# JuliaQuantumControl/Krotov.jl

Measured on NVIDIA B200. Metric: state_timesteps_per_s, higher is better.
Workload: dtype f64

## Files before the change

include/krotov_cuda.h:

```cpp
#ifndef KROTOV_CUDA_H
#define KROTOV_CUDA_H

#include <stdint.h>

#ifdef __cplusplus
extern "C" {
#endif

#define KROTOV_ABI_VERSION 1

typedef struct krotov_handle_s *krotov_handle;

enum krotov_status {
    KROTOV_OK = 0,
    KROTOV_ERR_ARG = 1,
    KROTOV_ERR_CUDA = 2,
    KROTOV_ERR_STATE = 3,
    KROTOV_ERR_UNSUPPORTED = 4,
    KROTOV_ERR_TIMEOUT = 5,
    KROTOV_ERR_NOMEM = 6
};

enum krotov_gen_format {
    KROTOV_GEN_DENSE_COLMAJOR = 0,
// ... 70 lines not shown
int krotov_create(const krotov_problem *problem, krotov_handle *out);
int krotov_destroy(krotov_handle h);
const char *krotov_last_error(krotov_handle h);
int krotov_get_info(krotov_handle h, krotov_info *out);

int krotov_set_cheby(krotov_handle h, int direction, int n_dt_class, const int32_t *dt_class_of_step,
                     const double *dt_of_class, const double *E_min, const double *Delta, const int32_t *m,
                     const double *coeffs, int m_max);

int krotov_set_amplitudes(krotov_handle h, int degree, const double *poly, const double *shape);

int krotov_forward(krotov_handle h, const double *pulses );

int krotov_set_chi(krotov_handle h, const double *chi );
int krotov_set_chi_coeffs(krotov_handle h, const double *coef);

int krotov_iterate(krotov_handle h, const double *guess_pulses, double *new_pulses, double *g_a_int);

int krotov_get_states(krotov_handle h, double *states );
int krotov_get_tau(krotov_handle h, double *tau );
int krotov_get_storage(krotov_handle h, int which, int k, int n0, int n1, double *out);

int krotov_get_profile(krotov_handle h, int cta, int64_t *out);

#define KROTOV_COMM_DESC_BYTES 256
int krotov_comm_export(krotov_handle h, void *desc );
int krotov_comm_connect(krotov_handle h, int rank, int world, const void *descs );

int krotov_group_connect(krotov_handle *handles, int world);
int krotov_group_iterate(krotov_handle *handles, int world, const double *guess_pulses, double *new_pulses,
                         double *g_a_int);

int krotov_hermitian_extremes(int n_mat, int d, const double *mats, double *e_min, double *e_max, int n_threads);
int krotov_envelope_extremes(int n_gen, int d, int n_ctrl, const double *H0, const double *Hc, int n_corner,
                             const double *amps, double *e_min, double *e_max, int n_threads);

int krotov_envelope_extremes_device(krotov_handle h, int n_corner, const double *amps, double *e_min, double *e_max);

#ifdef __cplusplus
}
#endif
#endif
```

krotov.jl_b200/_lib.py:

```python
from __future__ import annotations

import ctypes as C
import os

_HERE = os.path.dirname(os.path.abspath(__file__))
LIB_PATH = os.environ.get("KROTOV_CUDA_LIB") or os.path.join(_HERE, "libkrotov_cuda.so")

KROTOV_OK = 0
ERR_NAMES = {1: "KROTOV_ERR_ARG", 2: "KROTOV_ERR_CUDA", 3: "KROTOV_ERR_STATE", 4: "KROTOV_ERR_UNSUPPORTED",
             5: "KROTOV_ERR_TIMEOUT", 6: "KROTOV_ERR_NOMEM"}
GEN_DENSE_COLMAJOR, GEN_CSR = 0, 1
FORWARD, BACKWARD = 0, 1
CHI_HOST, CHI_SM, CHI_SS, CHI_RE = 0, 1, 2, 3
PATH_WARP, PATH_DENSE, PATH_SPARSE = 1, 2, 3
COMM_DESC_BYTES = 256

EXPORTS = [
    "krotov_abi_version", "krotov_create", "krotov_destroy", "krotov_last_error", "krotov_get_info",
    "krotov_set_cheby", "krotov_set_amplitudes", "krotov_forward", "krotov_set_chi", "krotov_set_chi_coeffs", "krotov_iterate",
    "krotov_get_states", "krotov_get_tau", "krotov_get_storage", "krotov_get_profile", "krotov_comm_export", "krotov_comm_connect",
    "krotov_group_connect", "krotov_group_iterate",
    "krotov_hermitian_extremes", "krotov_envelope_extremes", "krotov_envelope_extremes_device",
]


class KrotovCudaError(RuntimeError):
    def __init__(self, code, msg):
        super().__init__(f"libkrotov_cuda: {ERR_NAMES.get(code, code)}: {msg}")
        self.code = code
        self.detail = msg


class Problem(C.Structure):
    _fields_ = [
        ("struct_size", C.c_int32), ("d", C.c_int32), ("n_traj", C.c_int32), ("n_ctrl", C.c_int32),
        ("n_steps", C.c_int32), ("n_gen", C.c_int32), ("gen_format", C.c_int32), ("nnz", C.c_int32),
        ("tlist", C.c_void_p), ("gen_of_traj", C.c_void_p), ("csr_rowptr", C.c_void_p), ("csr_colind", C.c_void_p),
        ("gen_values", C.c_void_p), ("term_present", C.c_void_p), ("psi0", C.c_void_p), ("target", C.c_void_p),
        ("weight", C.c_void_p), ("update_shape", C.c_void_p), ("lambda_a", C.c_void_p),
        ("functional", C.c_int32), ("n_traj_global", C.c_int32), ("store_fw", C.c_int32), ("device", C.c_int32),
        ("force_path", C.c_int32), ("replicated_forward", C.c_int32), ("reserved", C.c_int32 * 6),
    ]

# ... 19 lines not shown
    if not os.path.exists(LIB_PATH):
        raise ImportError(
            f"{LIB_PATH} not found: the CUDA extension is not built. Run "
            "`python -c 'import __graft_entry__ as g; g.build()'` at the repo root. "
            "krotov_jl_b200 has no CPU fallback.")
    L = C.CDLL(LIB_PATH)
    vp, i32, dbl = C.c_void_p, C.c_int, C.c_double
    L.krotov_abi_version.restype = i32
    L.krotov_create.argtypes = [C.POINTER(Problem), C.POINTER(vp)]
    L.krotov_destroy.argtypes = [vp]
    L.krotov_last_error.argtypes = [vp]
    L.krotov_last_error.restype = C.c_char_p
    L.krotov_get_info.argtypes = [vp, C.POINTER(Info)]
    L.krotov_set_cheby.argtypes = [vp, i32, i32, vp, vp, vp, vp, vp, vp, i32]
    L.krotov_set_amplitudes.argtypes = [vp, i32, vp, vp]
    L.krotov_forward.argtypes = [vp, vp]
    L.krotov_set_chi.argtypes = [vp, vp]
    L.krotov_set_chi_coeffs.argtypes = [vp, vp]
    L.krotov_iterate.argtypes = [vp, vp, vp, vp]
    L.krotov_get_states.argtypes = [vp, vp]
    L.krotov_get_tau.argtypes = [vp, vp]
    L.krotov_get_storage.argtypes = [vp, i32, i32, i32, i32, vp]
    L.krotov_get_profile.argtypes = [vp, i32, vp]
    L.krotov_comm_export.argtypes = [vp, vp]
    L.krotov_comm_connect.argtypes = [vp, i32, i32, vp]
    L.krotov_group_connect.argtypes = [vp, i32]
    L.krotov_group_iterate.argtypes = [vp, i32, vp, vp, vp]
    L.krotov_hermitian_extremes.argtypes = [i32, i32, vp, vp, vp, i32]
    L.krotov_envelope_extremes.argtypes = [i32, i32, i32, vp, vp, i32, vp, vp, vp, i32]
    L.krotov_envelope_extremes_device.argtypes = [vp, i32, vp, vp, vp]
    for name in EXPORTS:
        if name not in ("krotov_last_error",):
            getattr(L, name).restype = i32
    L.krotov_last_error.restype = C.c_char_p
    _lib = L
    return L


def hermitian_extremes(stack, n_threads=0):
    import numpy as np

    a = np.ascontiguousarray(stack, np.complex128)
    n, d = a.shape[0], a.shape[-1]
    lo, hi = np.empty(n, np.float64), np.empty(n, np.float64)
    rc = lib().krotov_hermitian_extremes(n, d, a.ctypes.data_as(C.c_void_p), lo.ctypes.data_as(C.c_void_p),
                                         hi.ctypes.data_as(C.c_void_p), int(n_threads))
# ... 21 lines not shown
```

krotov.jl_b200/csrc/krotov_cuda.cu:

```cuda
#include <cuda_runtime.h>

#include <algorithm>
#include <chrono>
#include <cmath>
#include <complex>
#include <cstdio>
#include <cstdlib>
#include <cstring>
#include <map>
#include <set>
#include <string>
#include <vector>

#include <thread>

#include "../../include/krotov_cuda.h"
#include "dense_kernel.cuh"
#include "warp_kernel.cuh"
#include "warp2_kernel.cuh"
#include "tiny_kernel.cuh"
#include "kernel_table.h"

using cplx = std::complex<double>;

// ... 969 lines not shown
        if (h->has_target) {
            pad_states(pb->target, tmp);
            if ((rc = upload(h, h->d_target, tmp))) return bail(rc);
        }
        const size_t slab = (size_t)N * (N_T + 1) * h->lpt * 16;
        h->x_slab = slab / 16;
        if ((rc = dev_alloc(h, h->d_X, slab * (h->rf_wanted ? 2 : 1)))) return bail(rc);
        if (h->store_fw && (rc = dev_alloc(h, h->d_Phi, slab))) return bail(rc);
        if ((rc = dev_alloc(h, h->d_chiT, (size_t)N * h->lpt * 16))) return bail(rc);
        if ((rc = dev_alloc(h, h->d_psif, (size_t)N * h->lpt * 16))) return bail(rc);
        cudaMemcpy(h->d_psif.p, h->d_psi0.p, (size_t)N * h->lpt * 16, cudaMemcpyDeviceToDevice);
        if (h->has_target) {
            std::vector<cplx> tau0(N);
            const cplx *s0 = reinterpret_cast<const cplx *>(pb->psi0), *tg = reinterpret_cast<const cplx *>(pb->target);
            for (int k = 0; k < N; ++k) {
                cplx a(0, 0);
                for (int i = 0; i < d; ++i) a += std::conj(tg[(size_t)k * d + i]) * s0[(size_t)k * d + i];
                tau0[k] = a;
            }
            cudaMemcpy(h->d_tau.p, tau0.data(), (size_t)N * 16, cudaMemcpyHostToDevice);
        }
        h->swept = true;
        if ((rc = dev_alloc(h, h->d_R, ((size_t)N_T * h->nCTA * L + (size_t)N_T * L) * 8))) return bail(rc);
        if ((rc = dev_alloc(h, h->d_acc, (size_t)N_T * L * kr::kFixLimbs * 8))) return bail(rc);
        if (getenv("KROTOV_PROF")) {
            if ((rc = dev_alloc(h, h->d_prof, (size_t)h->nCTA * 8 * 8))) return bail(rc);
            cudaMemset(h->d_prof.p, 0, h->d_prof.bytes);
        }
    } else {
        kr::SparseDesc sd;
        if (path == KROTOV_PATH_SPARSE) {
            sd.W = hs.W; sd.nnz_union = hs.nnz_union; sd.hermitian = hs.hermitian;
            sd.cols = &hs.cols; sd.vals_f = &hs.vals_f; sd.vals_b = &hs.vals_b;
        }
        h->dense = kr::dense_create(h->d, h->N, h->L, h->N_T, h->n_gen, h->Hdense, h->gen_of_traj, pb->psi0,
                                    pb->target, h->store_fw, h->stream, h->err,
                                    path == KROTOV_PATH_SPARSE ? &sd : nullptr);
        if (!h->dense) return bail(KROTOV_ERR_UNSUPPORTED);
        std::vector<cplx>().swap(h->Hdense);
        if (!kr::dense_seed(h->dense, (double2 *)h->d_tau.p, h->err)) return bail(KROTOV_ERR_CUDA);
        h->swept = true;
    }
    if (cudaDeviceSynchronize() != cudaSuccess) return bail(fail(h, KROTOV_ERR_CUDA, "device sync after create failed"));
    *out = h;
    return KROTOV_OK;
}

int krotov_get_info(krotov_handle h, krotov_info *out) {
    if (!h || !out) return KROTOV_ERR_ARG;
// ... 537 lines not shown
            lo = std::min(lo, out[2 * ((size_t)g * n_corner + c)]);
            hi = std::max(hi, out[2 * ((size_t)g * n_corner + c) + 1]);
        }
        e_min[g] = lo;
        e_max[g] = hi;
    }
    return KROTOV_OK;
}

int krotov_get_profile(krotov_handle h, int cta, int64_t *out) {
    if (!h || !out) return KROTOV_ERR_ARG;
    for (int i = 0; i < 8; ++i) out[i] = 0;
    if (!h->d_prof.p) return fail(h, KROTOV_ERR_STATE, "profiling counters are off (set KROTOV_PROF=1 before krotov_create)");
    cudaSetDevice(h->device);
    std::vector<long long> tmp((size_t)h->nCTA * 8);
    KR_CUDA(h, cudaMemcpy(tmp.data(), h->d_prof.p, tmp.size() * 8, cudaMemcpyDeviceToHost));
    if (cta >= h->nCTA) return fail(h, KROTOV_ERR_ARG, "cta out of range");
    for (int c = 0; c < h->nCTA; ++c)
        if (cta < 0 || c == cta)
            for (int i = 0; i < 8; ++i) out[i] = std::max<int64_t>(out[i], tmp[(size_t)c * 8 + i]);
    return KROTOV_OK;
}

struct CommDesc {
    cudaIpcMemHandle_t mh[2];
    cudaIpcMemHandle_t xh;
};
struct CommDescTail {
    int nCTA;
    int n_traj, n_traj_global;
    int rf_ok;
};
static_assert(sizeof(CommDesc) + sizeof(CommDescTail) <= KROTOV_COMM_DESC_BYTES, "descriptor too large");

int krotov_comm_export(krotov_handle h, void *desc) {
    if (!h || !desc) return KROTOV_ERR_ARG;
    cudaSetDevice(h->device);
    CommDesc cd;
    memset(&cd, 0, sizeof(cd));
    for (int par = 0; par < 2; ++par) KR_CUDA(h, cudaIpcGetMemHandle(&cd.mh[par], h->d_mbox[par].p));
    if (h->path == KROTOV_PATH_WARP) KR_CUDA(h, cudaIpcGetMemHandle(&cd.xh, h->d_X.p));
    memset(desc, 0, KROTOV_COMM_DESC_BYTES);
    memcpy(desc, &cd, sizeof(cd));
    CommDescTail tail{h->path == KROTOV_PATH_WARP ? h->nCTA : 0, h->N, h->N_global, rf_eligible(h) ? 1 : 0};
    memcpy((char *)desc + sizeof(cd), &tail, sizeof(tail));
    return KROTOV_OK;
// ... 61 lines not shown
```

krotov.jl_b200/csrc/warp2_kernel.cuh:

```cuda
#pragma once
#include "warp_kernel.cuh"

namespace kr {

template <int W>
__device__ __forceinline__ void row_dot2(const double2 (&g)[W + 1], const int (&col)[W], const double2 *__restrict__ va,
                                         const double2 *__restrict__ vb, const double2 owna, const double2 ownb,
                                         double &ara, double &aia, double &arb, double &aib) {
    double ra1 = 0.0, ia1 = 0.0, rb1 = 0.0, ib1 = 0.0;
    ara = fma(g[W].x, owna.x, ara);
    ra1 = fma(-g[W].y, owna.y, ra1);
    aia = fma(g[W].x, owna.y, aia);
    ia1 = fma(g[W].y, owna.x, ia1);
    arb = fma(g[W].x, ownb.x, arb);
    rb1 = fma(-g[W].y, ownb.y, rb1);
    aib = fma(g[W].x, ownb.y, aib);
    ib1 = fma(g[W].y, ownb.x, ib1);
#pragma unroll
    for (int s = 0; s < W; ++s) {
        const double2 xa = va[col[s]];
        const double2 xb = vb[col[s]];
        ara = fma(g[s].x, xa.x, ara);
        ra1 = fma(-g[s].y, xa.y, ra1);
        aia = fma(g[s].x, xa.y, aia);
// ... 157 lines not shown
    StepMeta fmeta = load_meta(p.dtc_f, p.m_f, p.phase_f, p.coef_f, p.ndtc_f, p.mmax_f, gi, 0);
    double2 chia = make_double2(0.0, 0.0), chib = make_double2(0.0, 0.0);
    if (p.mode == 1 && live) {
        chia = p.X[(size_t)ka * (N_T + 1) * 32 + lane];
        chib = p.X[(size_t)kb * (N_T + 1) * 32 + lane];
    }
    long long t_wait_b = 0, t_overlap = 0, t_step = 0;
    for (int n = 0; n < N_T; ++n) {
        double eps[LT];
        const long long ts0 = clock64();
        if (p.mode == 1) {
            double part[LT];
#pragma unroll
            for (int l = 0; l < LT; ++l) part[l] = 0.0;
            if (live) {
#pragma unroll
                for (int l = 0; l < LT; ++l) {
                    double war = 0.0, wai = 0.0, wbr = 0.0, wbi = 0.0;
                    row_dot2<W>(P[l + 1], col, myps, myps + 32, pa, pb, war, wai, wbr, wbi);
                    part[l] = fma(inv_s, fma(chia.x, war, chia.y * wai), part[l]);
                    part[l] = fma(inv_s, fma(chib.x, wbr, chib.y * wbi), part[l]);
                }
            }
#pragma unroll
            for (int l = 0; l < LT; ++l) red[(size_t)l * wpc * 32 + warp * 32 + lane] = part[l];
            bar_arrive(1, nthr_all);
            const long long w0 = clock64();
            t_overlap += w0 - ts0;
            if (n + 1 < N_T && live) {
                chia = p.X[((size_t)ka * (N_T + 1) + n + 1) * 32 + lane];
                chib = p.X[((size_t)kb * (N_T + 1) + n + 1) * 32 + lane];
            }
            bar_sync(2, nthr_all);
#pragma unroll
            for (int l = 0; l < LT; ++l) eps[l] = eps_s[l];
            if (p.prof != nullptr) {
                asm volatile("" ::"d"(eps[0]) : "memory");
                t_wait_b += clock64() - w0;
            }
        } else {
#pragma unroll
            for (int l = 0; l < LT; ++l) eps[l] = p.amp_old[(size_t)l * N_T + n];
        }
        const StepMeta fmeta_next =
            load_meta(p.dtc_f, p.m_f, p.phase_f, p.coef_f, p.ndtc_f, p.mmax_f, gi, n + 1 < N_T ? n + 1 : n);
        if (live) {
#pragma unroll
            for (int s = 0; s <= W; ++s) g[s] = P[0][s];
// ... 56 lines not shown
```

krotov.jl_b200/csrc/warp_kernel.cuh:

```cuda
#pragma once
#include <cuda_runtime.h>
#include <stdint.h>

namespace kr {

constexpr int kMaxRanks = 8;
constexpr int kMaxCtrl = 8;
constexpr int kAmpMaxDeg = 4;
constexpr unsigned long long kSentinel = 0xFFFFFFFFFFFFFFFFull;

struct WarpParams {
    int d, N, L, N_T, n_gen;
    int wpc;
    int tpw;
    int nCTA;
    int mode;
    int mu_hermitian;
    int store_fw;
    int ndtc_f, ndtc_b, mmax_f, mmax_b;
    const int *gen_of_traj;
    const int *cols;
    const double2 *Pf, *Pb;
    const double *inv_s_f;
    const double *coef_f, *coef_b;
// ... 279 lines not shown

__device__ __forceinline__ void poll_broadcast(const double *E, const int L, const int lane, double (&tot)[kMaxCtrl],
                                               int *err_flag, const long long timeout) {
    const long long t0 = clock64();
    int spins = 0;
    unsigned long long u;
    for (;;) {
        u = ld_poll_u64<false>(E + (lane < L ? lane : 0));
        if (__all_sync(0xffffffffu, u != kSentinel)) break;
        if ((++spins & 63) == 0) {
            if (clock64() - t0 > timeout || *(volatile int *)err_flag) {
                atomicExch(err_flag, 1);
                break;
            }
        }
    }
    const double v = __longlong_as_double((long long)u);
#pragma unroll
    for (int l = 0; l < kMaxCtrl; ++l) tot[l] = __shfl_sync(0xffffffffu, v, l < L ? l : 0);
}


constexpr int kFixFrac = 88, kFixLimbBits = 40, kFixLimbs = 3, kFixBiasBit = 119;

__device__ __forceinline__ bool fix_from_double(const double x, unsigned __int128 &biased, const int lim_exp = 31) {
    const unsigned long long bits = (unsigned long long)__double_as_longlong(fabs(x));
    const int ebits = (int)(bits >> 52);
    if (ebits >= 1023 + lim_exp) return false;
    const unsigned long long mant = (bits & 0xFFFFFFFFFFFFFull) | (ebits ? (1ull << 52) : 0ull);
    const int shift = (ebits ? ebits : 1) - 1075 + kFixFrac;
    unsigned __int128 mag = 0;
    if (shift >= 0)
        mag = (unsigned __int128)mant << shift;
    else if (shift > -64)
        mag = mant >> (-shift);
    const unsigned __int128 bias = (unsigned __int128)1 << kFixBiasBit;
    biased = (x < 0.0) ? bias - mag : bias + mag;
    return true;
}

__device__ __forceinline__ double fix_to_double(const unsigned long long w0, const unsigned long long w1,
                                                const unsigned long long w2, const int n) {
    const unsigned long long mask = (1ull << 48) - 1;
    unsigned __int128 sum = (unsigned __int128)(w0 & mask) + ((unsigned __int128)(w1 & mask) << kFixLimbBits) +
                            ((unsigned __int128)(w2 & mask) << (2 * kFixLimbBits));
    const unsigned __int128 bias = (unsigned __int128)n << kFixBiasBit;
    const bool neg = sum < bias;
    const unsigned __int128 mag = neg ? bias - sum : sum - bias;
    const unsigned long long hi = (unsigned long long)(mag >> 64), lo = (unsigned long long)mag;
    double d;
    if (hi == 0) {
        d = __ull2double_rn(lo);
    } else {
        const int sh = 64 - __clzll((long long)hi);
        unsigned long long top = (sh == 64) ? hi : ((hi << (64 - sh)) | (lo >> sh));
        const unsigned long long lost = (sh == 64) ? lo : (lo << (64 - sh));
        if (lost) top |= 1ull;
        d = scalbn(__ull2double_rn(top), sh);
    }
    d = scalbn(d, -kFixFrac);
    return neg ? -d : d;
}

__device__ __forceinline__ void red_add_u64(unsigned long long *p, unsigned long long v) {
    asm volatile("red.relaxed.gpu.global.add.u64 [%0], %1;" ::"l"(p), "l"(v) : "memory");
}

__device__ __forceinline__ bool atomic_grid_sum(unsigned long long *An, const int nCTA, const int L, const int lane,
                                                double (&tot)[kMaxCtrl], int *err_flag, const long long timeout,
                                                const bool wait = true) {
    const int nw = L * kFixLimbs;
    const int myl = lane / kFixLimbs, myj = lane - myl * kFixLimbs;
    double mine = 0.0;
#pragma unroll
    for (int l = 0; l < kMaxCtrl; ++l)
        if (l == myl) mine = tot[l];
    if (lane < nw) {
        unsigned __int128 v;
        const bool ok = fix_from_double(mine, v);
        unsigned long long add = 1ull << 56;
        if (ok)
            add += (unsigned long long)(v >> (myj * kFixLimbBits)) & ((1ull << kFixLimbBits) - 1);
        else
            add += 1ull << 48;
        red_add_u64(An + lane, add);
    }
    if (!wait) return true;
    const long long t0 = clock64();
    int spins = 0;
    unsigned long long w = 0;
    for (;;) {
        if (lane < nw) w = ld_poll_u64<false>(reinterpret_cast<const double *>(An + lane));
        const bool pending = lane < nw && (int)(w >> 56) != nCTA;
        if (!__any_sync(0xffffffffu, pending)) break;
        if ((++spins & 63) == 0) {
            if (clock64() - t0 > timeout || *(volatile int *)err_flag) {
                atomicExch(err_flag, 1);
                break;
            }
        }
    }
    const bool misfit = lane < nw && ((w >> 48) & 0xFF) != 0;
    if (__any_sync(0xffffffffu, misfit)) return false;
    const int src = (lane < L ? lane : 0) * kFixLimbs;
    const unsigned long long w0 = __shfl_sync(0xffffffffu, w, src), w1 = __shfl_sync(0xffffffffu, w, src + 1),
                             w2 = __shfl_sync(0xffffffffu, w, src + 2);
    const double du = fix_to_double(w0, w1, w2, nCTA);
#pragma unroll
    for (int l = 0; l < kMaxCtrl; ++l) tot[l] = __shfl_sync(0xffffffffu, du, l < L ? l : 0);
    return true;
}

constexpr int kXLimbBits = 30, kXLimbs = 4, kXBiasBit = 116, kXMisShift = 41, kXCntShift = 52, kXMaxArrivals = 2047;

__device__ __forceinline__ bool fixx_from_double(const double x, unsigned __int128 &biased) {
    const unsigned long long bits = (unsigned long long)__double_as_longlong(fabs(x));
    const int ebits = (int)(bits >> 52);
    if (ebits >= 1023 + (kXBiasBit - kFixFrac)) return false;
    const unsigned long long mant = (bits & 0xFFFFFFFFFFFFFull) | (ebits ? (1ull << 52) : 0ull);
    const int shift = (ebits ? ebits : 1) - 1075 + kFixFrac;
    unsigned __int128 mag = 0;
    if (shift >= 0)
        mag = (unsigned __int128)mant << shift;
    else if (shift > -64)
        mag = mant >> (-shift);
    const unsigned __int128 bias = (unsigned __int128)1 << kXBiasBit;
    biased = (x < 0.0) ? bias - mag : bias + mag;
    return true;
}

__device__ __forceinline__ double fix_mag_to_double(const unsigned __int128 mag, const bool neg) {
    const unsigned long long hi = (unsigned long long)(mag >> 64), lo = (unsigned long long)mag;
    double d;
    if (hi == 0) {
        d = __ull2double_rn(lo);
    } else {
        const int sh = 64 - __clzll((long long)hi);
        unsigned long long top = (sh == 64) ? hi : ((hi << (64 - sh)) | (lo >> sh));
        const unsigned long long lost = (sh == 64) ? lo : (lo << (64 - sh));
        if (lost) top |= 1ull;
        d = scalbn(__ull2double_rn(top), sh);
    }
    d = scalbn(d, -kFixFrac);
    return neg ? -d : d;
}

__device__ __forceinline__ void red_add_sys_u64(unsigned long long *p, unsigned long long v) {
    asm volatile("red.relaxed.sys.global.add.u64 [%0], %1;" ::"l"(p), "l"(v) : "memory");
}

__device__ __forceinline__ bool xrank_atomic_sum(const WarpParams &p, const int n, const int L, const int lane,
                                                 double (&tot)[kMaxCtrl]) {
    const int nw = L * kXLimbs;
    const int myl = lane / kXLimbs, myj = lane - myl * kXLimbs;
    double mine = 0.0;
#pragma unroll
    for (int l = 0; l < kMaxCtrl; ++l)
        if (l == myl) mine = tot[l];
    const size_t off = ((size_t)n * nw + (lane < nw ? lane : 0)) * (size_t)p.xacc_stride;
    if (lane < nw) {
        unsigned __int128 v;
        const bool ok = fixx_from_double(mine, v);
        unsigned long long add = 1ull << kXCntShift;
        if (ok)
            add += (unsigned long long)(v >> (myj * kXLimbBits)) & ((1ull << kXLimbBits) - 1);
        else
            add += 1ull << kXMisShift;
// ... 16 lines not shown
                atomicExch(p.err_flag, 1);
                break;
            }
        }
    }
    const bool misfit = lane < nw && ((w >> kXMisShift) & 0x7FF) != 0;
    if (__any_sync(0xffffffffu, misfit)) return false;
    const int src = (lane < L ? lane : 0) * kXLimbs;
    const unsigned long long mask = (1ull << kXMisShift) - 1;
    unsigned __int128 sum = 0;
#pragma unroll
    for (int j = 0; j < kXLimbs; ++j)
        sum += (unsigned __int128)(__shfl_sync(0xffffffffu, w, src + j) & mask) << (j * kXLimbBits);
    const unsigned __int128 bias = (unsigned __int128)p.total_ctas << kXBiasBit;
    const bool neg = sum < bias;
    const double du = fix_mag_to_double(neg ? bias - sum : sum - bias, neg);
#pragma unroll
    for (int l = 0; l < kMaxCtrl; ++l) tot[l] = __shfl_sync(0xffffffffu, du, l < L ? l : 0);
    return true;
}

constexpr int kHSumBits = 52, kHMisShift = 52, kHCntShift = 56, kHLimExp = 28;

__device__ __forceinline__ unsigned long long atom_add_u64(unsigned long long *p, unsigned long long v) {
    unsigned long long old;
    asm volatile("atom.relaxed.gpu.global.add.u64 %0, [%1], %2;" : "=l"(old) : "l"(p), "l"(v) : "memory");
    return old;
}

__device__ __forceinline__ bool xrank_hier_sum(const WarpParams &p, const int n, const int L, const int lane,
                                               double (&tot)[kMaxCtrl]) {
    const int nw = L * kFixLimbs;
    const int myl = lane / kFixLimbs, myj = lane - myl * kFixLimbs;
    double mine = 0.0;
#pragma unroll
    for (int l = 0; l < kMaxCtrl; ++l)
        if (l == myl) mine = tot[l];
    const bool by_store = p.xchg_hier == 2;
    const size_t widx = ((size_t)n * L + (lane < nw ? myl : 0)) * kXLimbs + (lane < nw ? myj : 0);
    const size_t off = by_store ? widx * kMaxRanks : widx * (size_t)p.xacc_stride;
    if (lane < nw) {
        unsigned __int128 v;
        const bool ok = fix_from_double(mine, v, kHLimExp);
        unsigned long long add = 1ull << 56;
        if (ok)
            add += (unsigned long long)(v >> (myj * kFixLimbBits)) & ((1ull << kFixLimbBits) - 1);
        else
            add += 1ull << 48;
        unsigned long long total = add;
        if (p.nCTA > 1) total += atom_add_u64(p.acc + (size_t)n * nw + lane, add);
        if ((int)(total >> 56) == p.nCTA) {
            unsigned long long fwd = 1ull << kHCntShift;
            if ((total >> 48) & 0xFF)
                fwd += 1ull << kHMisShift;
            else
                fwd += total & ((1ull << 48) - 1);
            for (int i = 1; i <= p.world; ++i) {
                int r = p.rank + i;
                if (r >= p.world) r -= p.world;
                if (by_store)
                    asm volatile("st.relaxed.sys.global.u64 [%0], %1;" ::"l"(p.xacc[r] + off + p.rank), "l"(fwd) : "memory");
                else
                    red_add_sys_u64(p.xacc[r] + off, fwd);
            }
        }
    }
    const long long t0 = clock64();
    int spins = 0;
    unsigned long long w = 0;
    const double *mine_p = reinterpret_cast<const double *>(p.xacc[p.rank] + off);
    for (;;) {
        bool pending = false;
        if (lane < nw) {
// ... 42 lines not shown
    double tot[kMaxCtrl];
#pragma unroll
    for (int l = 0; l < kMaxCtrl; ++l) tot[l] = tot_io[l];
    bool summed = false, acc_used = false;
    if (p.xacc[0] != nullptr) {
        if (p.xchg_hier) {
            summed = xrank_hier_sum(p, n, L, lane, tot);
            acc_used = true;
        } else {
            summed = xrank_atomic_sum(p, n, L, lane, tot);
        }
        if (!summed && cta == 0 && lane == 0) atomicAdd(p.err_flag + 1, 1);
    }
    if (!summed) {
        double *Rn = p.R + (size_t)n * L * p.nCTA;
        const bool use_acc = p.acc != nullptr && p.nCTA > 1 && !acc_used;
        if (p.nCTA > 1) {
#pragma unroll
            for (int l = 0; l < kMaxCtrl; ++l)
                if (l < L && lane == l) st_relaxed_gpu_f64(Rn + (size_t)l * p.nCTA + cta, tot[l]);
        }
        bool have_rank_sum = p.nCTA == 1;
        if (use_acc)
            have_rank_sum = atomic_grid_sum(p.acc + (size_t)n * L * kFixLimbs, p.nCTA, L, lane, tot, p.err_flag,
                                            p.timeout_cycles, cta == 0);
        const size_t off = (size_t)n * L * p.world;
        if (cta == 0) {
            if (!have_rank_sum) {
                if (use_acc && lane == 0) atomicAdd(p.err_flag + 1, 1);
                reducer_gather<false>(Rn, p.nCTA, L, lane, gbuf, tot, p.err_flag, p.timeout_cycles);
            }
#pragma unroll
            for (int l = 0; l < kMaxCtrl; ++l)
                if (l < L && lane < p.world) st_relaxed_f64(p.mbox[lane] + off + (size_t)l * p.world + p.rank, tot[l]);
        }
        if (p.mbox_all || p.nCTA == 1) {
            reducer_gather<true>(p.mbox[p.rank] + off, p.world, L, lane, gbuf, tot, p.err_flag, p.timeout_cycles);
        } else {
            double *En = p.E + (size_t)n * L;
            if (cta == 0) {
                reducer_gather<true>(p.mbox[p.rank] + off, p.world, L, lane, gbuf, tot, p.err_flag, p.timeout_cycles);
#pragma unroll
                for (int l = 0; l < kMaxCtrl; ++l)
                    if (l < L && lane == l) st_relaxed_gpu_f64(En + l, tot[l]);
            } else {
                poll_broadcast(En, L, lane, tot, p.err_flag, p.timeout_cycles);
            }
// ... 19 lines not shown
    } else {
#pragma unroll
        for (int l = 0; l < kMaxCtrl; ++l)
            if (l < L && lane == l) st_relaxed_gpu_f64(Rn + (size_t)l * p.nCTA, tot[l]);
        reducer_gather<false>(Rn, p.nCTA, L, lane, gbuf, tot, p.err_flag, p.timeout_cycles);
#pragma unroll
        for (int l = 0; l < kMaxCtrl; ++l)
            if (l < L && lane == l) st_relaxed_gpu_f64(En + l, tot[l]);
    }
#pragma unroll
    for (int l = 0; l < kMaxCtrl; ++l) tot_io[l] = tot[l];
}

static __device__ __noinline__ double amp_eval_cold(const WarpParams *pp, const int l, const double e, const double shp) {
    double c = e;
    if (pp->amp_poly != nullptr) {
        const double *q = pp->amp_poly + l * (kAmpMaxDeg + 1);
        c = q[kAmpMaxDeg];
#pragma unroll
        for (int d = kAmpMaxDeg - 1; d >= 0; --d) c = fma(c, e, q[d]);
    }
    if (pp->amp_shape != nullptr) c = __dmul_rn(shp, c);
    return c;
}

__device__ __forceinline__ void comm_warp_run(const WarpParams &p, const int cta, const int L, const int lane, const int wpc,
                                              const int nthr_all, double *red, double *eps_s, double *gbuf,
                                              WarpParams *p_sh) {
    const int N_T = p.N_T;
    if (p.mode != 1) return;
    {
        const unsigned long long *src = reinterpret_cast<const unsigned long long *>(&p);
        unsigned long long *dst = reinterpret_cast<unsigned long long *>(p_sh);
        for (int i = lane; i < (int)(sizeof(WarpParams) / 8); i += 32) dst[i] = src[i];
        __syncwarp();
    }
    double ga = 0.0;
    const bool nonlin = p.amp_dfac != nullptr;
    long long c_wait_a = 0, c_reduce = 0, c_gather = 0;
    for (int n = 0; n < N_T; ++n) {
        double a_ln = 0.0, e_old = 0.0, dtn = 0.0, dfac = 1.0, shp = 1.0, a_eff = 0.0;
        if (lane < L) {
            a_ln = p.alpha[(size_t)lane * N_T + n];
            e_old = p.eps_old[(size_t)lane * N_T + n];
            dtn = p.dt[n];
            a_eff = a_ln;
            if (nonlin) {
                dfac = p.amp_dfac[(size_t)lane * N_T + n];
                if (p.amp_shape != nullptr) shp = p.amp_shape[(size_t)lane * N_T + n];
                a_eff = __dmul_rn(a_ln, dfac);
            }
        }
        const long long c0 = clock64();
        bar_sync(1, nthr_all);
        const long long c1 = clock64();
        double tot[kMaxCtrl];
#pragma unroll
        for (int l = 0; l < kMaxCtrl; ++l) {
            double sacc = 0.0;
            if (l < L)
                for (int q = 0; q < wpc; ++q) sacc += red[(size_t)l * wpc * 32 + q * 32 + lane];
            tot[l] = sacc;
        }
#pragma unroll
        for (int o = 16; o > 0; o >>= 1) {
#pragma unroll
            for (int l = 0; l < kMaxCtrl; ++l)
                if (l < L) tot[l] += __shfl_xor_sync(0xffffffffu, tot[l], o);
        }
        const long long c2 = clock64();
        bool summed = p.nCTA == 1 && p.world == 1;
        if (p.world > 1) {
            double tl[kMaxCtrl];
#pragma unroll
            for (int l = 0; l < kMaxCtrl; ++l) tl[l] = tot[l];
            exchange_ranks(p_sh, cta, n, L, lane, tl, gbuf);
#pragma unroll
            for (int l = 0; l < kMaxCtrl; ++l) tot[l] = tl[l];
            summed = true;
        } else if (p.acc != nullptr && p.nCTA > 1) {
            summed = atomic_grid_sum(p.acc + (size_t)n * L * kFixLimbs, p.nCTA, L, lane, tot, p.err_flag, p.timeout_cycles);
            if (!summed && cta == 0 && lane == 0) atomicAdd(p.err_flag + 1, 1);
        }
        if (!summed) {
            double tl[kMaxCtrl];
#pragma unroll
            for (int l = 0; l < kMaxCtrl; ++l) tl[l] = tot[l];
            exchange_gather(p_sh, cta, n, L, lane, tl, gbuf);
#pragma unroll
            for (int l = 0; l < kMaxCtrl; ++l) tot[l] = tl[l];
        }
        const long long c3 = clock64();
        c_wait_a += c1 - c0;
        c_reduce += c2 - c1;
        c_gather += c3 - c2;
        double mine = 0.0;
#pragma unroll
        for (int l = 0; l < kMaxCtrl; ++l)
            if (lane == l) mine = tot[l];
        double e_new = 0.0;
        if (lane < L) {
            const double d_eps = __dmul_rn(a_eff, mine);
            e_new = __dadd_rn(e_old, d_eps);
            double c_new = e_new;
            if (nonlin) c_new = amp_eval_cold(p_sh, lane, e_new, shp);
            eps_s[lane] = c_new;
        }
        bar_arrive(2, nthr_all);
        if (cta == 0 && lane < L) {
            p.eps_new[(size_t)lane * N_T + n] = e_new;
            const double du = nonlin ? __dmul_rn(dfac, mine) : mine;
            ga = __dadd_rn(ga, __dmul_rn(__dmul_rn(a_ln, __dmul_rn(fabs(du), fabs(du))), dtn));
        }
    }
    if (cta == 0 && lane < L) p.g_a_int[lane] = ga;
    if (p.prof != nullptr && lane == 0) {
        p.prof[cta * 8 + 3] = c_wait_a;
        p.prof[cta * 8 + 4] = c_reduce;
        p.prof[cta * 8 + 5] = c_gather;
    }
}

static __device__ __noinline__ void rf_forward_records(const WarpParams *pp, const double2 *rf_ring, unsigned long long *rf_bar,
                                                       int *rf_prog, const int cta, const int warp, const int lane,
                                                       const int n_prod, const int n_fwd) {
    const WarpParams &p = *pp;
    const int N_T = p.N_T, wpc = p.wpc, world = p.rf_world, nCTA = p.nCTA, bw_lo = p.bw_lo;
    const long long timeout = p.timeout_cycles;
    double2 *Xr[kMaxRanks];
#pragma unroll
    for (int r = 0; r < kMaxRanks; ++r) Xr[r] = p.Xr[r];
// ... 318 lines not shown
                const int k = kbase + t;
                if (k >= p.N) break;
                const int gi = (t == 0) ? g0 : p.gen_of_traj[k];
                const double inv_s = (t == 0) ? inv_s0 : p.inv_s_f[gi];
                const double2 psi = (tpw == 1) ? psi_reg : mypsi[t * LPT + lane];
                const double2 chi = (t == 0) ? chi_next : p.X[((size_t)k * (N_T + 1) + n) * LPT + lane];
                if (PREG) {
#pragma unroll
                    for (int l = 0; l < NT - 1; ++l) {
                        double wr = 0.0, wi = 0.0;
                        row_dot<W>(P[l + 1], col, mypsi + t * LPT, psi, wr, wi);
                        part[l] = fma(inv_s, fma(chi.x, wr, chi.y * wi), part[l]);
                    }
                } else {
                    const double2 *Pg = p.Pf + (size_t)gi * (1 + L) * rowstride;
                    for (int l = 0; l < L; ++l) {
                        load_row<W, LPT>(Pg + (size_t)(l + 1) * rowstride, g, lane);
                        double wr = 0.0, wi = 0.0;
                        row_dot<W>(g, col, mypsi + t * LPT, psi, wr, wi);
                        part[l] = fma(inv_s, fma(chi.x, wr, chi.y * wi), part[l]);
                    }
                }
            }
#pragma unroll
            for (int l = 0; l < (PREG ? LT : kMaxCtrl); ++l)
                if (l < L) red[(size_t)l * wpc * LPT + warp * LPT + lane] = part[l];
            bar_arrive(1, nthr_all);
            const long long w0 = clock64();
            t_overlap += w0 - ts0;
            if (n + 1 < N_T && k0 < p.N) chi_next = p.X[((size_t)k0 * (N_T + 1) + n + 1) * LPT + lane];
            if (PREG && FAST && k0 < p.N) {
#pragma unroll
                for (int q = 0; q < NT; ++q) {
                    double wr = 0.0, wi = 0.0;
                    row_dot<W>(P[q], col, mypsi, psi_reg, wr, wi);
                    wv[q] = make_double2(wr, wi);
                }
                chibuf[lane] = chi_next;
                grp_sync<LPT>(gbar);
#pragma unroll
                for (int l = 0; l < NT - 1; ++l) {
                    double wr = 0.0, wi = 0.0;
                    row_dot<W>(P[l + 1], col, chibuf, chi_next, wr, wi);
                    xi[l] = make_double2(wr, wi);
                }
                grp_sync<LPT>(gbar);
            }
            bar_sync(2, nthr_all);
#pragma unroll
            for (int l = 0; l < (PREG ? LT : kMaxCtrl); ++l)
                if (l < L) eps[l] = eps_s[l];
            if (p.prof != nullptr) {
                asm volatile("" ::"d"(eps[0]) : "memory");
                t_wait_b += clock64() - w0;
            }
        } else {
#pragma unroll
            for (int l = 0; l < (PREG ? LT : kMaxCtrl); ++l)
                if (l < L) eps[l] = p.amp_old[(size_t)l * N_T + n];
        }
        const StepMeta fmeta_next =
            load_meta(p.dtc_f, p.m_f, p.phase_f, p.coef_f, p.ndtc_f, p.mmax_f, g0, n + 1 < N_T ? n + 1 : n);
        for (int t = 0; t < tpw; ++t) {
            const int k = kbase + t;
            if (k >= p.N) break;
            const int gi = (t == 0) ? g0 : p.gen_of_traj[k];
            const StepMeta sm = (t == 0) ? fmeta : load_meta(p.dtc_f, p.m_f, p.phase_f, p.coef_f, p.ndtc_f, p.mmax_f, gi, n);
            if (PREG) {
#pragma unroll
                for (int s = 0; s <= W; ++s) g[s] = P[0][s];
#pragma unroll
                for (int l = 0; l < NT - 1; ++l) {
#pragma unroll
                    for (int s = 0; s <= W; ++s) {
                        g[s].x = fma(eps[l], P[l + 1][s].x, g[s].x);
                        g[s].y = fma(eps[l], P[l + 1][s].y, g[s].y);
                    }
// ... 80 lines not shown
```

krotov.jl_b200/engine.py:

```python
from __future__ import annotations

import ctypes as C

import numpy as np

from . import _lib as B


def _ptr(a):
    return None if a is None else a.ctypes.data_as(C.c_void_p)


class KrotovCuda:
    def __init__(self, *, tlist, H0, Hc, gen_of_traj, psi0, target=None, weight=None, update_shape, lambda_a,
                 functional=B.CHI_HOST, n_traj_global=0, store_fw=False, device=0, force_path=0, csr=False,
                 replicated_forward=False):
        lib = B.lib()
        self._lib = lib
        self._h = C.c_void_p()
        tlist = np.ascontiguousarray(tlist, np.float64)
        psi0 = np.ascontiguousarray(psi0, np.complex128)
        N, d = psi0.shape
        n_gen = len(H0)
        L = len(Hc[0])
# ... 133 lines not shown
    def tau(self):
        out = np.empty(self.N, np.complex128)
        self._check(self._lib.krotov_get_tau(self._h, _ptr(out)))
        return out

    def storage(self, which, k, n0=0, n1=None):
        n1 = self.N_T + 1 if n1 is None else n1
        out = np.empty((n1 - n0, self.d), np.complex128)
        self._check(self._lib.krotov_get_storage(self._h, int(which), int(k), int(n0), int(n1), _ptr(out)))
        return out

    def envelope_extremes(self, corners):
        amps = np.ascontiguousarray(corners, np.float64).reshape(-1, self.L)
        lo, hi = np.empty(self.n_gen, np.float64), np.empty(self.n_gen, np.float64)
        self._check(self._lib.krotov_envelope_extremes_device(self._h, amps.shape[0], _ptr(amps), _ptr(lo), _ptr(hi)))
        return lo, hi

    def profile(self, cta=-1):
        out = np.zeros(8, np.int64)
        self._check(self._lib.krotov_get_profile(self._h, int(cta), _ptr(out)))
        names = ["backward", "forward", "wait_pulse", "comm_wait_partials", "comm_reduce", "comm_gather", "overlap", "fw_step_total"]
        return dict(zip(names, out.tolist()))

    def comm_export(self):
        buf = (C.c_ubyte * B.COMM_DESC_BYTES)()
        self._check(self._lib.krotov_comm_export(self._h, buf))
        return bytes(buf)

    def comm_connect(self, rank, world, descs):
        blob = b"".join(descs)
        assert len(blob) == world * B.COMM_DESC_BYTES
        buf = (C.c_ubyte * len(blob)).from_buffer_copy(blob)
        self._check(self._lib.krotov_comm_connect(self._h, int(rank), int(world), buf))


class KrotovCudaGroup:

    def __init__(self, engines, bounds, gens, replicated=False):
        self.engines, self.bounds, self.gens = list(engines), list(bounds), [np.asarray(g, int) for g in gens]
        self.replicated = bool(replicated)
        e0 = self.engines[0]
        self._lib = e0._lib
        self.N = e0.N if replicated else sum(e.N for e in self.engines)
        self.d, self.L, self.N_T = e0.d, e0.L, e0.N_T
        self.n_gen = len(self.gens[0]) if replicated else sum(len(g) for g in self.gens)
        self.world = len(self.engines)
# ... 85 lines not shown
```

Measured before the change: 333.5 million.

## Warp-reduce partials before handoff and poll limbs directly in grid sum

Worker warps now reduce their per-control partials with warp shuffles before writing them to shared memory. The comm warp therefore sums one value per warp instead of 32 lanes per warp, and its trailing shuffle reduction is removed. The atomic grid sum has each lane poll its own three limbs directly rather than having many lanes poll and then shuffle, and the final broadcast is skipped where it is not needed. A per-step timeline profiler gated by KROTOV_PROF is also added; it adds clock reads when enabled and makes some parts of the code path differ from the unprofiled one.

```diff
diff --git a/include/krotov_cuda.h b/include/krotov_cuda.h
--- a/include/krotov_cuda.h
+++ b/include/krotov_cuda.h
@@ -116,6 +116,7 @@
 int krotov_get_storage(krotov_handle h, int which, int k, int n0, int n1, double *out);
 
 int krotov_get_profile(krotov_handle h, int cta, int64_t *out);
+int krotov_get_step_timeline(krotov_handle h, int64_t *out);
 
 #define KROTOV_COMM_DESC_BYTES 256
 int krotov_comm_export(krotov_handle h, void *desc );
diff --git a/krotov.jl_b200/_lib.py b/krotov.jl_b200/_lib.py
--- a/krotov.jl_b200/_lib.py
+++ b/krotov.jl_b200/_lib.py
@@ -18,7 +18,7 @@
 EXPORTS = [
     "krotov_abi_version", "krotov_create", "krotov_destroy", "krotov_last_error", "krotov_get_info",
     "krotov_set_cheby", "krotov_set_amplitudes", "krotov_forward", "krotov_set_chi", "krotov_set_chi_coeffs", "krotov_iterate",
-    "krotov_get_states", "krotov_get_tau", "krotov_get_storage", "krotov_get_profile", "krotov_comm_export", "krotov_comm_connect",
+    "krotov_get_states", "krotov_get_tau", "krotov_get_storage", "krotov_get_profile", "krotov_get_step_timeline", "krotov_comm_export", "krotov_comm_connect",
     "krotov_group_connect", "krotov_group_iterate",
     "krotov_hermitian_extremes", "krotov_envelope_extremes", "krotov_envelope_extremes_device",
 ]
@@ -84,6 +84,7 @@
     L.krotov_get_tau.argtypes = [vp, vp]
     L.krotov_get_storage.argtypes = [vp, i32, i32, i32, i32, vp]
     L.krotov_get_profile.argtypes = [vp, i32, vp]
+    L.krotov_get_step_timeline.argtypes = [vp, vp]
     L.krotov_comm_export.argtypes = [vp, vp]
     L.krotov_comm_connect.argtypes = [vp, i32, i32, vp]
     L.krotov_group_connect.argtypes = [vp, i32]
diff --git a/krotov.jl_b200/csrc/krotov_cuda.cu b/krotov.jl_b200/csrc/krotov_cuda.cu
--- a/krotov.jl_b200/csrc/krotov_cuda.cu
+++ b/krotov.jl_b200/csrc/krotov_cuda.cu
@@ -1015,9 +1015,9 @@
         }
         h->swept = true;
         if ((rc = dev_alloc(h, h->d_R, ((size_t)N_T * h->nCTA * L + (size_t)N_T * L) * 8))) return bail(rc);
-        if ((rc = dev_alloc(h, h->d_acc, (size_t)N_T * L * kr::kFixLimbs * 8))) return bail(rc);
+        if ((rc = dev_alloc(h, h->d_acc, (size_t)N_T * kr::acc_step_words(L) * 8))) return bail(rc);
         if (getenv("KROTOV_PROF")) {
-            if ((rc = dev_alloc(h, h->d_prof, (size_t)h->nCTA * 8 * 8))) return bail(rc);
+            if ((rc = dev_alloc(h, h->d_prof, (size_t)h->nCTA * (8 + kr::kTlSamples * kr::kTlSlots) * 8))) return bail(rc);
             cudaMemset(h->d_prof.p, 0, h->d_prof.bytes);
         }
     } else {
@@ -1601,6 +1601,15 @@
     return KROTOV_OK;
 }
 
+int krotov_get_step_timeline(krotov_handle h, int64_t *out) {
+    if (!h || !out) return KROTOV_ERR_ARG;
+    if (!h->d_prof.p) return fail(h, KROTOV_ERR_STATE, "profiling counters are off (set KROTOV_PROF=1 before krotov_create)");
+    cudaSetDevice(h->device);
+    const size_t n = (size_t)h->nCTA * kr::kTlSamples * kr::kTlSlots;
+    KR_CUDA(h, cudaMemcpy(out, (const long long *)h->d_prof.p + (size_t)h->nCTA * 8, n * 8, cudaMemcpyDeviceToHost));
+    return KROTOV_OK;
+}
+
 struct CommDesc {
     cudaIpcMemHandle_t mh[2];
     cudaIpcMemHandle_t xh;
diff --git a/krotov.jl_b200/csrc/warp2_kernel.cuh b/krotov.jl_b200/csrc/warp2_kernel.cuh
--- a/krotov.jl_b200/csrc/warp2_kernel.cuh
+++ b/krotov.jl_b200/csrc/warp2_kernel.cuh
@@ -203,8 +203,7 @@
                     part[l] = fma(inv_s, fma(chib.x, wbr, chib.y * wbi), part[l]);
                 }
             }
-#pragma unroll
-            for (int l = 0; l < LT; ++l) red[(size_t)l * wpc * 32 + warp * 32 + lane] = part[l];
+            hand_over_partials(part, LT, red, wpc, warp, lane);
             bar_arrive(1, nthr_all);
             const long long w0 = clock64();
             t_overlap += w0 - ts0;
diff --git a/krotov.jl_b200/csrc/warp_kernel.cuh b/krotov.jl_b200/csrc/warp_kernel.cuh
--- a/krotov.jl_b200/csrc/warp_kernel.cuh
+++ b/krotov.jl_b200/csrc/warp_kernel.cuh
@@ -325,6 +325,14 @@
 
 
 constexpr int kFixFrac = 88, kFixLimbBits = 40, kFixLimbs = 3, kFixBiasBit = 119;
+constexpr int kAccWordStride = 1;
+__host__ __device__ constexpr size_t acc_step_words(const int L) { return (size_t)L * kFixLimbs * kAccWordStride; }
+
+constexpr int kTlEvery = 16, kTlSamples = 128, kTlSlots = 16;
+__device__ __forceinline__ long long *tl_record(const WarpParams &p, const int cta, const int n) {
+    if (p.prof == nullptr || n % kTlEvery != 0 || n / kTlEvery >= kTlSamples) return nullptr;
+    return p.prof + (size_t)p.nCTA * 8 + ((size_t)cta * kTlSamples + n / kTlEvery) * kTlSlots;
+}
 
 __device__ __forceinline__ bool fix_from_double(const double x, unsigned __int128 &biased, const int lim_exp = 31) {
     const unsigned long long bits = (unsigned long long)__double_as_longlong(fabs(x));
@@ -342,6 +350,20 @@
     return true;
 }
 
+__device__ __forceinline__ double fix_mag_to_double(const unsigned __int128 mag, const bool neg) {
+    const unsigned long long hi = (unsigned long long)(mag >> 64), lo = (unsigned long long)mag;
+    const int sh = hi ? 64 - __clzll((long long)hi) : 0;
+    unsigned long long top = lo;
+    if (sh == 64) {
+        top = hi | (lo != 0 ? 1ull : 0ull);
+    } else if (sh > 0) {
+        top = (hi << (64 - sh)) | (lo >> sh);
+        if (lo << (64 - sh)) top |= 1ull;
+    }
+    const double d = __ull2double_rn(top) * __longlong_as_double((long long)(1023 + sh - kFixFrac) << 52);
+    return neg ? -d : d;
+}
+
 __device__ __forceinline__ double fix_to_double(const unsigned long long w0, const unsigned long long w1,
                                                 const unsigned long long w2, const int n) {
     const unsigned long long mask = (1ull << 48) - 1;
@@ -349,35 +371,29 @@
                             ((unsigned __int128)(w2 & mask) << (2 * kFixLimbBits));
     const unsigned __int128 bias = (unsigned __int128)n << kFixBiasBit;
     const bool neg = sum < bias;
-    const unsigned __int128 mag = neg ? bias - sum : sum - bias;
-    const unsigned long long hi = (unsigned long long)(mag >> 64), lo = (unsigned long long)mag;
-    double d;
-    if (hi == 0) {
-        d = __ull2double_rn(lo);
-    } else {
-        const int sh = 64 - __clzll((long long)hi);
-        unsigned long long top = (sh == 64) ? hi : ((hi << (64 - sh)) | (lo >> sh));
-        const unsigned long long lost = (sh == 64) ? lo : (lo << (64 - sh));
-        if (lost) top |= 1ull;
-        d = scalbn(__ull2double_rn(top), sh);
-    }
-    d = scalbn(d, -kFixFrac);
-    return neg ? -d : d;
+    return fix_mag_to_double(neg ? bias - sum : sum - bias, neg);
 }
 
 __device__ __forceinline__ void red_add_u64(unsigned long long *p, unsigned long long v) {
     asm volatile("red.relaxed.gpu.global.add.u64 [%0], %1;" ::"l"(p), "l"(v) : "memory");
 }
 
+__device__ __forceinline__ unsigned long long atom_add_u64(unsigned long long *p, unsigned long long v) {
+    unsigned long long old;
+    asm volatile("atom.relaxed.gpu.global.add.u64 %0, [%1], %2;" : "=l"(old) : "l"(p), "l"(v) : "memory");
+    return old;
+}
+
 __device__ __forceinline__ bool atomic_grid_sum(unsigned long long *An, const int nCTA, const int L, const int lane,
                                                 double (&tot)[kMaxCtrl], int *err_flag, const long long timeout,
-                                                const bool wait = true) {
+                                                const bool wait = true, const bool bcast = true, long long *tl = nullptr) {
     const int nw = L * kFixLimbs;
     const int myl = lane / kFixLimbs, myj = lane - myl * kFixLimbs;
     double mine = 0.0;
 #pragma unroll
     for (int l = 0; l < kMaxCtrl; ++l)
         if (l == myl) mine = tot[l];
+    unsigned long long prev = 0;
     if (lane < nw) {
         unsigned __int128 v;
         const bool ok = fix_from_double(mine, v);
@@ -386,15 +402,24 @@
             add += (unsigned long long)(v >> (myj * kFixLimbBits)) & ((1ull << kFixLimbBits) - 1);
         else
             add += 1ull << 48;
-        red_add_u64(An + lane, add);
-    }
+        if (tl != nullptr && lane == 0)
+            prev = atom_add_u64(An, add);
+        else
+            red_add_u64(An + lane * kAccWordStride, add);
+    }
+    if (tl != nullptr && lane == 0) tl[2] = clock64();
     if (!wait) return true;
+    const int src = lane < L ? lane * kFixLimbs : 0;
     const long long t0 = clock64();
     int spins = 0;
-    unsigned long long w = 0;
+    unsigned long long w0 = 0, w1 = 0, w2 = 0;
     for (;;) {
-        if (lane < nw) w = ld_poll_u64<false>(reinterpret_cast<const double *>(An + lane));
-        const bool pending = lane < nw && (int)(w >> 56) != nCTA;
+        if (lane < L) {
+            w0 = ld_poll_u64<false>(reinterpret_cast<const double *>(An + (src + 0) * kAccWordStride));
+            w1 = ld_poll_u64<false>(reinterpret_cast<const double *>(An + (src + 1) * kAccWordStride));
+            w2 = ld_poll_u64<false>(reinterpret_cast<const double *>(An + (src + 2) * kAccWordStride));
+        }
+        const bool pending = lane < L && ((int)(w0 >> 56) != nCTA || (int)(w1 >> 56) != nCTA || (int)(w2 >> 56) != nCTA);
         if (!__any_sync(0xffffffffu, pending)) break;
         if ((++spins & 63) == 0) {
             if (clock64() - t0 > timeout || *(volatile int *)err_flag) {
@@ -403,14 +428,15 @@
             }
         }
     }
-    const bool misfit = lane < nw && ((w >> 48) & 0xFF) != 0;
+    if (tl != nullptr && lane == 0) {
+        tl[3] = clock64();
+        tl[5] = (long long)(prev >> 56);
+    }
+    const bool misfit = lane < L && (((w0 | w1 | w2) >> 48) & 0xFF) != 0;
     if (__any_sync(0xffffffffu, misfit)) return false;
-    const int src = (lane < L ? lane : 0) * kFixLimbs;
-    const unsigned long long w0 = __shfl_sync(0xffffffffu, w, src), w1 = __shfl_sync(0xffffffffu, w, src + 1),
-                             w2 = __shfl_sync(0xffffffffu, w, src + 2);
     const double du = fix_to_double(w0, w1, w2, nCTA);
 #pragma unroll
-    for (int l = 0; l < kMaxCtrl; ++l) tot[l] = __shfl_sync(0xffffffffu, du, l < L ? l : 0);
+    for (int l = 0; l < kMaxCtrl; ++l) tot[l] = bcast ? __shfl_sync(0xffffffffu, du, l < L ? l : 0) : du;
     return true;
 }
 
@@ -430,22 +456,6 @@
     const unsigned __int128 bias = (unsigned __int128)1 << kXBiasBit;
     biased = (x < 0.0) ? bias - mag : bias + mag;
     return true;
-}
-
-__device__ __forceinline__ double fix_mag_to_double(const unsigned __int128 mag, const bool neg) {
-    const unsigned long long hi = (unsigned long long)(mag >> 64), lo = (unsigned long long)mag;
-    double d;
-    if (hi == 0) {
-        d = __ull2double_rn(lo);
-    } else {
-        const int sh = 64 - __clzll((long long)hi);
-        unsigned long long top = (sh == 64) ? hi : ((hi << (64 - sh)) | (lo >> sh));
-        const unsigned long long lost = (sh == 64) ? lo : (lo << (64 - sh));
-        if (lost) top |= 1ull;
-        d = scalbn(__ull2double_rn(top), sh);
-    }
-    d = scalbn(d, -kFixFrac);
-    return neg ? -d : d;
 }
 
 __device__ __forceinline__ void red_add_sys_u64(unsigned long long *p, unsigned long long v) {
@@ -508,12 +518,6 @@
 
 constexpr int kHSumBits = 52, kHMisShift = 52, kHCntShift = 56, kHLimExp = 28;
 
-__device__ __forceinline__ unsigned long long atom_add_u64(unsigned long long *p, unsigned long long v) {
-    unsigned long long old;
-    asm volatile("atom.relaxed.gpu.global.add.u64 %0, [%1], %2;" : "=l"(old) : "l"(p), "l"(v) : "memory");
-    return old;
-}
-
 __device__ __forceinline__ bool xrank_hier_sum(const WarpParams &p, const int n, const int L, const int lane,
                                                double (&tot)[kMaxCtrl]) {
     const int nw = L * kFixLimbs;
@@ -534,7 +538,7 @@
         else
             add += 1ull << 48;
         unsigned long long total = add;
-        if (p.nCTA > 1) total += atom_add_u64(p.acc + (size_t)n * nw + lane, add);
+        if (p.nCTA > 1) total += atom_add_u64(p.acc + (size_t)n * acc_step_words(L) + lane * kAccWordStride, add);
         if ((int)(total >> 56) == p.nCTA) {
             unsigned long long fwd = 1ull << kHCntShift;
             if ((total >> 48) & 0xFF)
@@ -623,7 +627,7 @@
         }
         bool have_rank_sum = p.nCTA == 1;
         if (use_acc)
-            have_rank_sum = atomic_grid_sum(p.acc + (size_t)n * L * kFixLimbs, p.nCTA, L, lane, tot, p.err_flag,
+            have_rank_sum = atomic_grid_sum(p.acc + (size_t)n * acc_step_words(L), p.nCTA, L, lane, tot, p.err_flag,
                                             p.timeout_cycles, cta == 0);
         const size_t off = (size_t)n * L * p.world;
         if (cta == 0) {
@@ -689,6 +693,31 @@
     }
     if (pp->amp_shape != nullptr) c = __dmul_rn(shp, c);
     return c;
+}
+
+template <int NL>
+__device__ __forceinline__ void hand_over_partials(double (&part)[NL], const int L, double *red, const int nw32,
+                                                   const int hw, const int lane32) {
+    if constexpr (NL == kMaxCtrl) {
+        for (int l = 0; l < L; ++l) {
+            double v = part[l];
+#pragma unroll
+            for (int o = 16; o > 0; o >>= 1) v += __shfl_xor_sync(0xffffffffu, v, o);
+            if (lane32 == 0) red[(size_t)l * nw32 + hw] = v;
+        }
+    } else {
+#pragma unroll
+        for (int o = 16; o > 0; o >>= 1) {
+#pragma unroll
+            for (int l = 0; l < NL; ++l)
+                if (l < L) part[l] += __shfl_xor_sync(0xffffffffu, part[l], o);
+        }
+        if (lane32 == 0) {
+#pragma unroll
+            for (int l = 0; l < NL; ++l)
+                if (l < L) red[(size_t)l * nw32 + hw] = part[l];
+        }
+    }
 }
 
 __device__ __forceinline__ void comm_warp_run(const WarpParams &p, const int cta, const int L, const int lane, const int wpc,
@@ -718,24 +747,36 @@
                 a_eff = __dmul_rn(a_ln, dfac);
             }
         }
+        long long *const rec = tl_record(p, cta, n);
         const long long c0 = clock64();
         bar_sync(1, nthr_all);
         const long long c1 = clock64();
+        if (rec != nullptr) {
+            const double x = red[0];
+            asm volatile("" ::"d"(x) : "memory");
+            if (lane == 0) rec[0] = clock64();
+        }
         double tot[kMaxCtrl];
 #pragma unroll
         for (int l = 0; l < kMaxCtrl; ++l) {
             double sacc = 0.0;
-            if (l < L)
-                for (int q = 0; q < wpc; ++q) sacc += red[(size_t)l * wpc * 32 + q * 32 + lane];
+            if (l < L) {
+                const double *r = red + (size_t)l * wpc;
+                for (int q0 = 0; q0 < wpc; q0 += 8) {
+                    double v[8];
+#pragma unroll
+                    for (int j = 0; j < 8; ++j) v[j] = (q0 + j < wpc) ? r[q0 + j] : 0.0;
+#pragma unroll
+                    for (int j = 0; j < 8; ++j) sacc += v[j];
+                }
+            }
             tot[l] = sacc;
         }
-#pragma unroll
-        for (int o = 16; o > 0; o >>= 1) {
-#pragma unroll
-            for (int l = 0; l < kMaxCtrl; ++l)
-                if (l < L) tot[l] += __shfl_xor_sync(0xffffffffu, tot[l], o);
-        }
         const long long c2 = clock64();
+        if (rec != nullptr && lane == 0) {
+            asm volatile("" ::"d"(tot[0]) : "memory");
+            rec[1] = clock64();
+        }
         bool summed = p.nCTA == 1 && p.world == 1;
         if (p.world > 1) {
             double tl[kMaxCtrl];
@@ -746,7 +787,8 @@
             for (int l = 0; l < kMaxCtrl; ++l) tot[l] = tl[l];
             summed = true;
         } else if (p.acc != nullptr && p.nCTA > 1) {
-            summed = atomic_grid_sum(p.acc + (size_t)n * L * kFixLimbs, p.nCTA, L, lane, tot, p.err_flag, p.timeout_cycles);
+            summed = atomic_grid_sum(p.acc + (size_t)n * acc_step_words(L), p.nCTA, L, lane, tot, p.err_flag,
+                                     p.timeout_cycles, true, false, rec);
             if (!summed && cta == 0 && lane == 0) atomicAdd(p.err_flag + 1, 1);
         }
         if (!summed) {
@@ -774,6 +816,7 @@
             eps_s[lane] = c_new;
         }
         bar_arrive(2, nthr_all);
+        if (rec != nullptr && lane == 0) rec[4] = clock64();
         if (cta == 0 && lane < L) {
             p.eps_new[(size_t)lane * N_T + n] = e_new;
             const double du = nonlin ? __dmul_rn(dfac, mine) : mine;
@@ -1138,9 +1181,7 @@
                     }
                 }
             }
-#pragma unroll
-            for (int l = 0; l < (PREG ? LT : kMaxCtrl); ++l)
-                if (l < L) red[(size_t)l * wpc * LPT + warp * LPT + lane] = part[l];
+            hand_over_partials(part, L, red, wpc * (LPT / 32), (warp * LPT + lane) >> 5, lane & 31);
             bar_arrive(1, nthr_all);
             const long long w0 = clock64();
             t_overlap += w0 - ts0;
@@ -1162,13 +1203,25 @@
                 }
                 grp_sync<LPT>(gbar);
             }
+            long long t_pre = 0;
+            if (p.prof != nullptr) {
+                if (PREG && FAST) asm volatile("" ::"d"(xi[0].x) : "memory");
+                t_pre = clock64();
+            }
             bar_sync(2, nthr_all);
 #pragma unroll
             for (int l = 0; l < (PREG ? LT : kMaxCtrl); ++l)
                 if (l < L) eps[l] = eps_s[l];
             if (p.prof != nullptr) {
                 asm volatile("" ::"d"(eps[0]) : "memory");
-                t_wait_b += clock64() - w0;
+                const long long t_eps = clock64();
+                t_wait_b += t_eps - w0;
+                long long *const rec = tl_record(p, cta, n);
+                if (rec != nullptr && warp == 0 && lane == 0) {
+                    rec[6] = w0;
+                    rec[7] = t_pre;
+                    rec[8] = t_eps;
+                }
             }
         } else {
 #pragma unroll
diff --git a/krotov.jl_b200/engine.py b/krotov.jl_b200/engine.py
--- a/krotov.jl_b200/engine.py
+++ b/krotov.jl_b200/engine.py
@@ -179,6 +179,14 @@
         names = ["backward", "forward", "wait_pulse", "comm_wait_partials", "comm_reduce", "comm_gather", "overlap", "fw_step_total"]
         return dict(zip(names, out.tolist()))
 
+    TIMELINE_EVERY, TIMELINE_SAMPLES, TIMELINE_SLOTS = 16, 128, 16
+
+    def step_timeline(self):
+        n = int(self.info()["grid_blocks"])
+        out = np.zeros((n, self.TIMELINE_SAMPLES, self.TIMELINE_SLOTS), np.int64)
+        self._check(self._lib.krotov_get_step_timeline(self._h, _ptr(out)))
+        return out
+
     def comm_export(self):
         buf = (C.c_ubyte * B.COMM_DESC_BYTES)()
         self._check(self._lib.krotov_comm_export(self._h, buf))
```

Result: slower. 317.4 million (median of 6 runs) (-4.8%).
